# marinlauber/WaterLily

Hardware: AMD Instinct MI355X
Metric: MLUPS (cell-updates/s) per sim_step!, 3D sphere (higher is better)
Workload: dtype f32; 1 GPU; 3D sphere 512x512x512, Re=3700, f32, uniform inflow, remeasure=false (BASELINE configs[2]); layout=padded, transport=none, comm_ranks=1, scalar_allreduce=none

## Files before the change

### waterlily_amd/csrc/wl_api.hip

```cpp
#include <cstdarg>
#include <cstring>

#include <fcntl.h>
#include <sys/mman.h>
#include <sys/stat.h>
#include <unistd.h>

#include <rccl/rccl.h>

#include "wl_ops.h"
#include "wl_coarse.h"
#include "wl_measure.h"
#include "wl_mesh.h"
#include "wl_stats.h"
#include "wl_probe.h"
#include "wl_integrals.h"

namespace wl {

struct RcclComm : Comm {
    ncclComm_t nc = nullptr;
    ncclComm_t nch = nullptr;
    ~RcclComm() override {
        if (nch) ncclCommDestroy(nch);
// ... 177 lines not shown
};

Scratch &global_scratch(int *rc) {
    static Scratch s;
    static bool ok = false;
    *rc = 0;
    if (!ok) { *rc = s.init(); ok = (*rc == 0); }
    return s;
}

}

using namespace wl;

struct wl_mg {
    wl_dtype t;
    int D;
    int nlev;
    int permask;
    std::vector<wl_level_desc> lev;
    Scratch sc;
    std::vector<void *> rowc;
    unsigned char *dirty = nullptr;
    bool log_on = false;
    std::vector<double> log;
    int alloc_rowc() {
        const size_t es = t == WL_F32 ? 4 : 8;
        rowc.assign(nlev, nullptr);
        for (int l = 0; l < nlev; ++l) {
            const wl_grid &g = lev[l].g;
            if (g.D != 3) continue;
            WL_HIP(wl_dev_alloc(&rowc[l], (size_t)g.n[1] * (size_t)g.n[2] * RC_N * es));
        }
        return 0;
    }
    void free_scratch() {
        for (void *p : rowc) if (p) (void)hipFree(p);
        rowc.clear();
        if (dirty) (void)hipFree(dirty);
        dirty = nullptr;
    }
};
struct wl_flow {
    wl_dtype t;
    wl_flow_desc d;
    Scratch sc;
    unsigned char *rowfree = nullptr;
    unsigned char *rowbuf = nullptr;
    unsigned char *segbuf = nullptr;
    bool seg_valid = false;
    const unsigned char *segfree() const { return (seg_valid && opt(WL_OPT_BDIM_ROWFLAGS)) ? segbuf : nullptr; }
    int *busy = nullptr;
    int nbusy = 0;
    int nbusy_lo = 0, nbusy_hi = 0;
    size_t busy_cap = 0;
    int *rowcount = nullptr;
    long *rowoff = nullptr;
    unsigned char *touched = nullptr, *prev = nullptr;
    unsigned char *changed = nullptr;
    bool changed_valid = false;
    bool changed_pending = false;
    bool prev_valid = false;
    long nband = -1;
};

template <class T> static LevelT<T> lvl(const wl_mg *m, int l) {
    const wl_level_desc &d = m->lev[l];
    LevelT<T> o;
    o.g = mkG(&d.g);
    o.L = (T *)d.L; o.D = (T *)d.D; o.iD = (T *)d.iD; o.x = (T *)d.x; o.eps = (T *)d.eps; o.r = (T *)d.r; o.z = (T *)d.z;
    o.rowc = (opt(WL_OPT_ROW_CONST_L) && l < (int)m->rowc.size()) ? (const T *)m->rowc[l] : nullptr;
    return o;
}

template <class T, int D> static int mg_update(wl_mg *m, const unsigned char *dirty = nullptr) {
    {
        LevelT<T> p = lvl<T>(m, 0);
        WL_TRY((op_set_diag<T, D>(p.g, p.D, p.iD, p.L, dirty)));
        WL_TRY((halo_exchange<T>(p.g, p.iD, 1, 1)));
        if (D == 3 && m->rowc[0]) WL_TRY((op_lrow<T>(p.g, p.L, p.iD, (T *)m->rowc[0], dirty)));
    }
    for (int l = 1; l < m->nlev; ++l) {
        LevelT<T> a = lvl<T>(m, l), b = lvl<T>(m, l - 1);
        WL_TRY((op_restrictL<T, D>(a.g, a.L, b.g, b.L, m->permask)));
        WL_TRY((coarse_L_finish<T, D>(a.g, a.L, b.g, m->permask)));
        WL_TRY((op_set_diag<T, D>(a.g, a.D, a.iD, a.L)));
        WL_TRY((halo_exchange<T>(a.g, a.iD, 1, 1)));
        if (D == 3 && m->rowc[l]) WL_TRY((op_lrow<T>(a.g, a.L, a.iD, (T *)m->rowc[l])));
    }
    return 0;
}

template <class T, int D> static int mg_vcycle(wl_mg *m, int l, int *pcg_np = nullptr) {
    LevelT<T> fine = lvl<T>(m, l), coarse = lvl<T>(m, l + 1);
    const bool fused = (m->permask == 0) && opt(WL_OPT_SMOOTH_FUSED);
    if (fused) WL_TRY((op_smooth_fused<T, D>(fine, fine.eps)));
    else WL_TRY((op_jacobi<T, D>(fine, 1, m->permask)));
    const bool zero_in_restrict = (m->permask == 0) && !coarse.g.dist && !fine.g.dist;
    WL_TRY((op_restrict<T, D>(coarse.g, coarse.r, fine.g, fused ? fine.eps : fine.r, zero_in_restrict ? coarse.x : (T *)nullptr)));
    if (ctx().comm && ctx().comm->size > 1 && fine.g.dist && !coarse.g.dist) {
        const int nzl = (fine.g.nzg - 2) / ctx().comm->size / 2;
        WL_TRY(ctx().comm->allgather(coarse.r + coarse.g.s[2], (size_t)nzl * coarse.g.s[2] * sizeof(T)));
    }
    if (!zero_in_restrict) {
        Prof p(WL_K_MISC, coarse.g.cells());
        WL_HIP(hipMemsetAsync(coarse.x, 0, (size_t)span(coarse.g) * sizeof(T), ctx().stream));
    }
    const long tail_cells = coarse_tail_cells();
    bool tail = tail_cells && fused && !coarse.g.dist && coarse.g.interior_cells() <= tail_cells && (m->nlev - (l + 1)) <= CV_MAXLEV;
    if (tail) {
        CoarseArgs<T> ca;
        ca.nlev = m->nlev - (l + 1);
        for (int q = 0; q < ca.nlev; ++q) {
            ca.lev[q] = lvl<T>(m, l + 1 + q);
            if (ca.lev[q].g.dist) tail = false;
        }
        if (tail) {
            Prof p(WL_K_SMOOTH, coarse.g.cells());
            if (opt(WL_OPT_COARSE_PCG_RESIDENT)) hipLaunchKernelGGL((k_coarse_vcycle<T, D, true>), dim3(1), dim3(CV_THREADS), 0, ctx().stream, ca);
            else hipLaunchKernelGGL((k_coarse_vcycle<T, D, false>), dim3(1), dim3(CV_THREADS), 0, ctx().stream, ca);
            WL_HIP(hipGetLastError());
        }
    }
    if (!tail) {
        int pre = -1;
        if (l + 2 < m->nlev) WL_TRY((mg_vcycle<T, D>(m, l + 1, pcg_np ? &pre : nullptr)));
        WL_TRY((op_pcg<T, D>(coarse, 6, m->permask, m->sc.partials, m->sc.st, false, pre)));
    }
    if (pcg_np) *pcg_np = -1;
    if (fused) return op_prolong_increment_fused<T, D>(fine, fine.eps, coarse.g, coarse.x, m->sc.partials, pcg_np);
    WL_TRY((op_prolongate<T, D>(fine.g, fine.eps, coarse.g, coarse.x)));
    return op_increment<T, D>(fine, m->permask);
}

template <class T, int D> static int mg_Linf(wl_mg *m, int l) {
    LevelT<T> p = lvl<T>(m, l);
    const T *r = p.r;
    return op_reduce<T, D>(p.g, WL_K_DOT, RED_MAX, 0.0, [=] __device__(long I) { const double v = (double)r[I]; return v < 0 ? -v : v; },
                           m->sc.partials, m->sc.st, 1, true);
}
template <class T, int D> static int mg_log_row(wl_mg *m, int n, bool have_r2) {
    if (!have_r2) WL_TRY((op_L2<T, D>(lvl<T>(m, 0), m->sc.partials, m->sc.st, false)));
    WL_TRY((mg_Linf<T, D>(m, 0)));
    WL_TRY(m->sc.fetch());
    m->log.push_back((double)n); m->log.push_back(m->sc.hst->out[1]); m->log.push_back(m->sc.hst->r2);
    return 0;
}
template <class T, int D> static int mg_solve(wl_mg *m, double tol, int itmx, int *n_iter, const T *divu = nullptr, const G *gu = nullptr,
                                              bool halo_begun = false) {
    LevelT<T> p = lvl<T>(m, 0);
    WL_TRY((op_residual<T, D>(p, m->permask, m->sc.partials, m->sc.st, divu, gu, halo_begun)));
    int n = 0;
    if (m->log_on) WL_TRY((mg_log_row<T, D>(m, 0, false)));
    while (n < itmx) {
        int pre = -1;
        if (m->nlev > 1) WL_TRY((mg_vcycle<T, D>(m, 0, &pre)));
        WL_TRY((op_pcg<T, D>(p, 6, m->permask, m->sc.partials, m->sc.st, true, pre, true)));
        WL_TRY((op_L2<T, D>(p, m->sc.partials, m->sc.st, true)));
        WL_TRY(m->sc.fetch());
        ++n;
        const double r2 = m->sc.hst->r2;
        if (m->log_on) WL_TRY((mg_log_row<T, D>(m, n, true)));
        if (r2 < tol) break;
    }
    WL_TRY((op_bc_per<T, D>(p.g, p.x, m->permask)));
    if (n_iter) *n_iter = n;
    return 0;
}

template <class T> static ScaleOp project_scale(double dt_, double w) {
    const bool dbl = (w != 1.0);
    return ScaleOp{dbl ? w * (double)(T)dt_ : (double)(T)dt_, false, dbl};
}
template <class T, int D> static int flow_project(wl_flow *a, wl_mg *b, double dt_, double w, int *n_iter, bool exchange_u = false,
                                                  bool head_done = false, const ScaleOp *tail_then = nullptr, const XBc<T> *xbc = nullptr,
                                                  bool *xdone = nullptr, T *uvel = nullptr) {
    const G g = mkG(&a->d.g);
    T *const uv = uvel ? uvel : (T *)a->d.u;
    LevelT<T> p = lvl<T>(b, 0);
    const ScaleOp sc = project_scale<T>(dt_, w);
// ... 821 lines not shown
                       m->dirty, gm.n[1], gm.n[2], (int)yper, (int)zper);
    WL_HIP(hipGetLastError());
    const unsigned char *dirty = m->dirty;
    WL_MG_DISPATCH((mg_update<T, DD>(m, dirty)));
}
int wl_mg_mult(wl_mg *m, int level, void *x) {
    WL_LEVEL_OK();
    WL_MG_DISPATCH((op_mult<T, DD>(lvl<T>(m, level), (T *)x, m->permask)));
}
int wl_mg_residual(wl_mg *m, int level) {
    WL_LEVEL_OK();
    WL_MG_DISPATCH((op_residual<T, DD>(lvl<T>(m, level), m->permask, m->sc.partials, m->sc.st)));
}
int wl_mg_increment(wl_mg *m, int level) {
    WL_LEVEL_OK();
    WL_MG_DISPATCH((op_increment<T, DD>(lvl<T>(m, level), m->permask)));
}
int wl_mg_jacobi(wl_mg *m, int level, int it) {
    WL_LEVEL_OK();
    WL_MG_DISPATCH((op_jacobi<T, DD>(lvl<T>(m, level), it, m->permask)));
}
int wl_mg_pcg(wl_mg *m, int level, int it, int *n_updates) {
    WL_LEVEL_OK();
    int rc = [&]() -> int { WL_MG_DISPATCH((op_pcg<T, DD>(lvl<T>(m, level), it, m->permask, m->sc.partials, m->sc.st, false, -1, level == 0))); }();
    if (rc) return rc;
    if (n_updates) {
        WL_TRY(m->sc.fetch());
        *n_updates = m->sc.hst->nupd;
    }
    return 0;
}
int wl_mg_uniform_rows(wl_mg *m, int level, long long *n_uniform, long long *n_rows) {
    WL_LEVEL_OK();
    if (!n_uniform || !n_rows) return fail(WL_E_ARG, "wl_mg_uniform_rows: null output", __FILE__, __LINE__);
    const wl_grid &g = m->lev[level].g;
    *n_uniform = 0;
    *n_rows = (long long)(g.n[1] - 2) * (g.D == 3 ? (g.own_hi > 0 ? g.own_hi - g.own_lo + 1 : g.n[2] - 2) : 1);
    if (g.D != 3 || level >= (int)m->rowc.size() || !m->rowc[level]) return 0;
    const size_t es = m->t == WL_F32 ? 4 : 8, cnt = (size_t)g.n[1] * g.n[2] * RC_N;
    std::vector<char> h(cnt * es);
    WL_HIP(hipMemcpyAsync(h.data(), m->rowc[level], cnt * es, hipMemcpyDeviceToHost, ctx().stream));
    WL_HIP(hipStreamSynchronize(ctx().stream));
    for (size_t r = 0; r < cnt; r += RC_N) {
        const double c = m->t == WL_F32 ? (double)reinterpret_cast<const float *>(h.data())[r] : reinterpret_cast<const double *>(h.data())[r];
        if (c == c) ++*n_uniform;
    }
    return 0;
// ... 430 lines not shown
```

### waterlily_amd/csrc/wl_ops.h

```cpp
#pragma once
#include "wl_common.h"
#include "wl_convdiff.h"
#include "wl_stencil7.h"

namespace wl {

struct State {
    double rho, alpha, beta;
    double shift;
    double r2;
    double out[4];
    double red[4];
    int active;
    int do_shift;
    int nupd;
    int r2_valid;
    int xpend;
    PcgS slots[2];
};

template <class T> struct LevelT {
    G g;
    T *L, *D, *iD, *x, *eps, *r, *z;
    const T *rowc = nullptr;
};

inline long span(const G &g) { return g.D == 3 ? (long)g.n[2] * g.s[2] : (long)g.n[1] * g.s[1]; }

template <class T, int D> int op_bc_vec_fused(const G &g, T *a, const double *A, int saveexit, int permask, bool skip_x = false);
template <class T> struct XBc { int on, saveexit; T U0; };
template <class T> __device__ __forceinline__ void xbc_apply(const XBc<T> &b, T *u, long o, long sc, int i, int n0, VecA<T> (&uv)[3]) {
    constexpr int V = VecA<T>::V;
    if (!b.on) return;
    if (i == 1) { uv[0].v[0] = b.U0; u[o - 1] = b.U0; u[o - 1 + sc] = uv[1].v[0]; u[o - 1 + 2 * sc] = uv[2].v[0]; }
    if (i + V - 1 == n0 - 2) {
        if (!b.saveexit) u[o + V] = b.U0;
        u[o + V + sc] = uv[1].v[V - 1]; u[o + V + 2 * sc] = uv[2].v[V - 1];
    }
}
template <class T, int D>
int op_bc_vec(const G &g, T *a, const double *A, int saveexit, int permask, bool skip_x = false) {
    if (opt(WL_OPT_BC_FUSED)) return op_bc_vec_fused<T, D>(g, a, A, saveexit, permask, skip_x);
    if (skip_x) return fail(WL_E_STATE, "BC!: x planes folded into the producer need the one-launch form", __FILE__, __LINE__);
    for (int c = 0; c < D; ++c)
        for (int j = 0; j < D; ++j) {
            T *ac = a + (long)c * g.sc;
            const long sj = g.s[j];
            const int N = (j == 2) ? g.nzg : g.n[j];
// ... 1050 lines not shown
    }
    if (!exchanged) WL_TRY((halo_exchange<T>(p.g, p.r, 1, 1)));
    return launch_range(WL_K_SMOOTH, r_inside(p.g), [=] __device__(int i, int j, int k) {
        const long I = q.g.at(i, j, k);
        T lo[D], hi[D];
_Pragma("unroll")
        for (int d = 0; d < D; ++d) { lo[d] = q.L[I + (long)d * q.g.sc]; hi[d] = q.L[I + q.g.s[d] + (long)d * q.g.sc]; }
        T dg = 0;
_Pragma("unroll")
        for (int d = 0; d < D; ++d) dg -= (lo[d] + hi[d]);
        const T e0 = q.r[I] * q.iD[I];
        T s = e0 * dg;
_Pragma("unroll")
        for (int d = 0; d < D; ++d) {
            const long sd = q.g.s[d];
            s += (q.r[I - sd] * q.iD[I - sd]) * lo[d] + (q.r[I + sd] * q.iD[I + sd]) * hi[d];
        }
        rout[I] = q.r[I] - s;
        q.x[I] = q.x[I] + e0;
    });
}
template <class T, int D>
int op_prolong_increment_fused(const LevelT<T> &p, const T *rin, const G &gc, const T *cx, double *partials = nullptr,
                               int *pcg_np = nullptr) {
    WL_TRY((halo_exchange<T>(gc, const_cast<T *>(cx), 1, 1)));
    const LevelT<T> q = p;
    const G C = gc;
    if (pcg_np) *pcg_np = -1;
    if constexpr (D == 3) {
        if (stencil7_ok<T>(p.g)) {
            using VA = VecA<T>;
            const SrcProlong<T> src{cx, C, p.g.n[0], p.g.n[1], p.g.nzg, p.g.kz0};
            if (pcg_np && partials && opt(WL_OPT_PCG_START_FUSED) && opt(WL_OPT_PCG_RECOMPUTE_PRECOND) && opt(WL_OPT_PCG_VEC)) {
                T *e0 = p.eps;
                const int tpp = (((p.g.n[0] - 2 + 64 * VA::V - 1) / (64 * VA::V)) * ((p.g.n[1] - 2 + 3) / 4) + 7) / 8 * 8;
                Gate gcap;
                if (tpp <= WL_PCG_PARTIALS) gcap.zcap = WL_PCG_PARTIALS / tpp;
                int np = 0;
                const int rcv = launch_stencil7<T, 1>(WL_K_PROLONG, p.g, src, p.L, p.rowc, rin, p.x,
                    [=] __device__(long o, int i, int, int, const VA &ae, const VA &ec, const VA &r0, const VA &x0, const auto &rk, double *acc, const Pre &) {
                        VA rv = r0, xv = x0;
                        const VA id = row_iD<T>(rk, q.iD, o, i, q.g.n[0]);
_Pragma("unroll")
                        for (int v = 0; v < VA::V; ++v) { rv.v[v] = rv.v[v] - ae.v[v]; xv.v[v] = xv.v[v] + ec.v[v]; }
                        rv.store(q.r + o);
                        xv.store(q.x + o);
                        VA ev;
_Pragma("unroll")
                        for (int v = 0; v < VA::V; ++v) { ev.v[v] = rv.v[v] * id.v[v]; acc[0] += (double)rv.v[v] * (double)ev.v[v]; }
                        ev.store(e0 + o);
                    }, partials, &np, gcap);
                if (rcv > 0) return rcv;
                if (rcv == 0) { *pcg_np = np; return 0; }
            }
            const int rcv = launch_stencil7<T, 0>(WL_K_PROLONG, p.g, src, p.L, p.rowc, rin, p.x,
                [=] __device__(long o, int, int, int, const VA &ae, const VA &ec, const VA &r0, const VA &x0, const auto &, double *, const Pre &) {
                    VA rv = r0, xv = x0;
// ... 44 lines not shown
        : form(f), st(st_), partials(partials_), dist(dist_), xdef(xdef_), want_r2(want_r2_), eps10(eps10_), f32(sizeof(T) == 4), zcap(zcap_) {
        const bool own = f != PcgForm::FINALIZE;
        P0 = partials; PA = own ? partials + WL_MAXB : partials; PB = own ? partials + 2 * WL_MAXB : partials;
    }
    Gate base() const { Gate g; g.eps10 = (double)eps10; g.f32 = f32; g.zcap = zcap; return g; }
    int ready(const double *&part, int &n) const {
        if (form != PcgForm::SLAB) return 0;
        Prof pr(WL_K_SCALAR, 0);
        WL_TRY((reduce_allreduce<1>(part, n, (int)RED_SUM, 0.0, st->red)));
        part = st->red;
        n = 1;
        return 0;
    }
    int after_init(int np) const {
        if (form != PcgForm::FINALIZE) return 0;
        State *s = st;
        const T e10 = eps10;
        return launch_finalize<1>(dist, partials, np, RED_SUM, 0.0, st->red, [=] __device__(const double *v) {
            const T rho = (T)v[0];
            s->rho = (double)rho;
            s->nupd = 0;
            s->r2_valid = 0;
            s->xpend = 0;
            s->active = !((rho < 0 ? -rho : rho) < e10);
        });
    }
    int gate_mult(int n, int np0, Gate &g) {
        g = base();
        if (form == PcgForm::FINALIZE) { g.active = &st->active; return 0; }
        if (n == 1) {
            const double *gp = P0; int gn = np0;
            WL_TRY(ready(gp, gn));
            g.kind = 1; g.part = gp; g.np = gn; g.out = &st->slots[0]; cur = 0;
        } else { g.kind = 4; g.in = &st->slots[cur]; }
        return 0;
    }
    int after_mult(int np) const {
        if (form != PcgForm::FINALIZE) return 0;
        State *s = st;
        return launch_finalize<1>(dist, partials, np, RED_SUM, 0.0, st->red, [=] __device__(const double *v) {
            s->xpend = 0;
            if (!s->active) return;
            const T alpha = (T)s->rho / (T)v[0];
            const double aa = (double)(alpha < 0 ? -alpha : alpha);
            s->alpha = (double)alpha;
            if (aa < 1e-2 || aa > 1e2) s->active = 0;
        });
    }
    int gate_update(int npA, Gate &g) {
        g = base();
        if (form == PcgForm::FINALIZE) { g.active = &st->active; g.s0 = &st->alpha; return 0; }
        const double *gp = PA; int gn = npA;
        WL_TRY(ready(gp, gn));
        g.kind = 2; g.part = gp; g.np = gn; g.in = &st->slots[cur]; g.out = &st->slots[cur ^ 1];
        return 0;
    }
    void launched_update() { if (form != PcgForm::FINALIZE) cur ^= 1; }
    int after_update(int np, bool last, bool xnow) const {
        State *s = st;
        const bool wr2 = want_r2;
        if (form != PcgForm::FINALIZE) {
            if (!last) return 0;
            const int cs = cur;
            return launch_finalize<1>(dist, PB, np, RED_SUM, 0.0, st->red, [=] __device__(const double *v) {
                PcgS sl = s->slots[cs];
                if (sl.active) {
                    sl.nupd += 1;
                    if (wr2) { sl.r2 = (double)(T)v[0]; sl.r2_valid = 1; }
                    sl.active = 0;
                }
                s->rho = sl.rho; s->alpha = sl.alpha; s->beta = sl.beta;
                s->active = sl.active; s->xpend = sl.xpend; s->nupd = sl.nupd;
                s->r2_valid = sl.r2_valid;
                if (sl.r2_valid) s->r2 = sl.r2;
            });
        }
        const T e10 = eps10;
        return launch_finalize<1>(dist, partials, np, RED_SUM, 0.0, st->red, [=] __device__(const double *v) {
            if (!s->active) return;
            s->nupd += 1;
            if (last) {
                if (wr2) { s->r2 = (double)(T)v[0]; s->r2_valid = 1; }
                s->active = 0;
                return;
            }
            const T rho2 = (T)v[0];
            if ((rho2 < 0 ? -rho2 : rho2) < e10) { s->active = 0; s->xpend = !xnow; return; }
            s->beta = (double)(rho2 / (T)s->rho);
            s->rho = (double)rho2;
        });
    }
    int gate_direction(int npB, Gate &g) {
        g = base();
        if (form == PcgForm::FINALIZE) {
            g.active = &st->active; g.also = xdef ? &st->xpend : nullptr; g.s0 = &st->alpha; g.s1 = &st->beta;
            return 0;
        }
        const double *gp = PB; int gn = npB;
        WL_TRY(ready(gp, gn));
        g.kind = 3; g.part = gp; g.np = gn; g.in = &st->slots[cur]; g.out = &st->slots[cur ^ 1]; g.also_x = 1;
        return 0;
    }
    void launched_direction() { if (form != PcgForm::FINALIZE) cur ^= 1; }
};

inline bool pcg_recompute_aeps(long cells) {
    const int v = opt(WL_OPT_PCG_RECOMPUTE_AEPS);
    return v == 2 || (v == 3 && cells < (1L << 26)) || (v == 1 && cells < (1L << 26) && cells >= (1L << 22));
}
inline bool pcg_dots_in_kernel(long cells, bool distr) {
    const int v = opt(WL_OPT_PCG_DOTS_IN_KERNEL);
    return distr ? v != 0 : (v == 2 || (v == 1 && cells <= (1L << 25)));
}

template <class T, int D>
int op_pcg(const LevelT<T> &p, int it, int permask, double *partials, State *st, bool want_r2 = false,
           int pre_np = -1,
           bool ghost_z = false) {
    const LevelT<T> q = p;
    const Range R = r_inside(p.g);
    using VA = VecA<T>;
    const int n0 = p.g.n[0];
    bool vec = false;
    if constexpr (D == 3) vec = pcg_vec_ok<T>(p.g);
    const bool xdef = opt(WL_OPT_PCG_DEFER_X) != 0;
    const bool zrec = opt(WL_OPT_PCG_RECOMPUTE_PRECOND) != 0;
    bool zst = false;
    if constexpr (D == 3) zst = pcg_recompute_aeps(R.count()) && vec && zrec;
    const int tpp_v = D == 3 ? (((p.g.n[0] - 2 + 64 * VA::V - 1) / (64 * VA::V)) * ((p.g.n[1] - 2 + 3) / 4) + 7) / 8 * 8 : 0;
    const bool distr = p.g.dist && ctx().comm && ctx().comm->size > 1;
    const bool gates = vec && xdef && zrec && R.count() > 0 && tpp_v > 0 && pcg_dots_in_kernel(R.count(), distr) &&
                       (distr || tpp_v <= WL_PCG_PARTIALS);
    const PcgForm form = !gates ? PcgForm::FINALIZE : (distr ? PcgForm::SLAB : PcgForm::IN_KERNEL);
    const int zcap = form == PcgForm::IN_KERNEL ? std::max(WL_PCG_PARTIALS / std::max(tpp_v, 1), 1) : 0;
    PcgDots<T> dots(form, st, partials, p.g.dist, xdef, want_r2, (T)10 * Lim<T>::eps, zcap);
    const bool own = form != PcgForm::FINALIZE;
    int np = 0, np0 = 0, npA = 0;

    int rv0 = -1;
    if (pre_np >= 0) { rv0 = 0; np = np0 = pre_np; }
    else if (vec) {
        Gate gate_init = dots.base();
        rv0 = launch_rowvec<T, 1, true>(WL_K_PCG_INIT, p.g,
            [=] __device__(long o, int, int, const Pre &) { return VA::load(q.r + o); },
            [=] __device__(long o, int i, int, int, const VA &rr, const auto &rk, double *acc, const Pre &) {
                const VA id = row_iD<T>(rk, q.iD, o, i, n0);
                VA zv;
_Pragma("unroll")
                for (int v = 0; v < VA::V; ++v) { zv.v[v] = rr.v[v] * id.v[v]; acc[0] += (double)rr.v[v] * (double)zv.v[v]; }
                if (!zrec) zv.store(q.z + o);
                zv.store(q.eps + o);
            }, p.rowc, dots.P0, &np, gate_init);
        if (rv0 > 0) return rv0;
        np0 = np;
    }
    if (own && rv0 != 0) return fail(WL_E_STATE, "pcg: vector init kernel rejected", __FILE__, __LINE__);
    if (rv0 != 0)
    WL_TRY((launch_range_red<1>(WL_K_PCG_INIT, R, [=] __device__(int i, int j, int k, double(&acc)[1]) {
        const long I = q.g.at(i, j, k);
        const T v = q.r[I] * q.iD[I];
        if (!zrec) q.z[I] = v;
        q.eps[I] = v;
        acc[0] += (double)q.r[I] * (double)v;
    }, partials, RED_SUM, 0.0, &np)));
    WL_TRY(dots.after_init(np));

    for (int n = 1; n <= it; ++n) {
        const bool last = (n == it);
        const bool xnow = last || !xdef;
        WL_TRY((op_bc_per<T, D>(p.g, p.eps, permask, false)));
        bool exchanged = false;
        int rcv = -1;
        if constexpr (D == 3) {
            if (stencil7_ok<T>(p.g)) {
                exchanged = true;
                Gate gate_mult;
                WL_TRY(dots.gate_mult(n, np0, gate_mult));
                rcv = launch_stencil7_halo<T, 1>(WL_K_PCG_MULT, p.g, p.eps, SrcArray<T>{p.eps}, p.L, p.rowc, (const T *)nullptr, (const T *)nullptr,
                    [=] __device__(long o, int, int, int, const VA &ae, const VA &ec, const VA &, const VA &, const auto &, double *acc, const Pre &) {
                    if (!zst) ae.store(q.z + o);
_Pragma("unroll")
                    for (int v = 0; v < VA::V; ++v) acc[0] += (double)ae.v[v] * (double)ec.v[v];
                }, dots.PA, &np, gate_mult);
                if (rcv > 0) return rcv;
                if (own && rcv != 0) return fail(WL_E_STATE, "pcg: vector mult kernel rejected", __FILE__, __LINE__);
            }
        }
        if (!exchanged) WL_TRY((halo_exchange<T>(p.g, p.eps, 1, 1)));
        if (rcv != 0)
        WL_TRY((launch_range_red<1>(WL_K_PCG_MULT, R, [=] __device__(int i, int j, int k, double(&acc)[1]) {
            if (!st->active) return;
            const long I = q.g.at(i, j, k);
            const T v = mult1r<T, D>(q.g, q.L, q.eps, I);
            q.z[I] = v;
            acc[0] += (double)v * (double)q.eps[I];
        }, partials, RED_SUM, 0.0, &np)));
        if (ghost_z && permask != 0) {
            int planes = 0, nps = 0;
            for (int j = 0; j < D; ++j) if ((permask >> j) & 1) planes |= 3 << (2 * j);
            const G gg = p.g;
            WL_TRY((launch_shell_red(WL_K_PCG_MULT, p.g, planes, [=] __device__(int i, int j, int k, double(&acc)[1]) {
                const long I = gg.at(i, j, k);
                acc[0] += (double)q.z[I] * (double)q.eps[I];
            }, (rcv == 0 ? dots.PA : partials) + np, RED_SUM, 0.0, &nps, own ? 32 : 256)));
            np += nps;
        }
        npA = np;
        WL_TRY(dots.after_mult(np));

        int rvu = -1;
        Gate gate_upd;
        WL_TRY(dots.gate_update(npA, gate_upd));
        if constexpr (D == 3) {
            if (zst) {
                auto upd_epi = [=] __device__(long o, int i, int, int, const VA &ae, const VA &ec, const VA &r0, const VA &x0, const auto &rk, double *acc, const Pre &pre) {
                    const T alpha = (T)pre.s0;
                    VA rr = r0;
                    if (xnow) {
                        VA xv = x0;
_Pragma("unroll")
                        for (int v = 0; v < VA::V; ++v) xv.v[v] += alpha * ec.v[v];
                        xv.store(q.x + o);
                    }
_Pragma("unroll")
                    for (int v = 0; v < VA::V; ++v) rr.v[v] = rr.v[v] - alpha * ae.v[v];
                    rr.store(q.r + o);
                    if (!last) {
                        const VA id = row_iD<T>(rk, q.iD, o, i, n0);
_Pragma("unroll")
                        for (int v = 0; v < VA::V; ++v) { const T zn = rr.v[v] * id.v[v]; acc[0] += (double)rr.v[v] * (double)zn; }
                    } else if (want_r2) {
_Pragma("unroll")
                        for (int v = 0; v < VA::V; ++v) acc[0] += (double)rr.v[v] * (double)rr.v[v];
                    }
                };
                const T *xin = xnow ? (const T *)q.x : (const T *)nullptr;
                rvu = launch_stencil7<T, 1>(WL_K_PCG_UPDATE, p.g, SrcArray<T>{p.eps}, p.L, p.rowc, (const T *)q.r, xin, upd_epi, dots.PB, &np, gate_upd);
                if (rvu != 0) return rvu > 0 ? rvu : fail(WL_E_STATE, "pcg: 7-point update kernel rejected", __FILE__, __LINE__);
                dots.launched_update();
            }
        }
        if (vec && rvu != 0) {
            struct UD { VA r, z, x, e; };
            rvu = launch_rowvec<T, 1, true>(WL_K_PCG_UPDATE, p.g,
                [=] __device__(long o, int, int, const Pre &) {
                    UD d;
                    d.r = VA::load(q.r + o);
                    d.z = VA::load(q.z + o);
                    if (xnow) { d.x = VA::load(q.x + o); d.e = VA::load(q.eps + o); }
                    return d;
                },
                [=] __device__(long o, int i, int, int, const UD &d, const auto &rk, double *acc, const Pre &pre) {
                    const T alpha = (T)pre.s0;
                    VA rr = d.r;
                    if (xnow) {
                        VA xv = d.x;
_Pragma("unroll")
                        for (int v = 0; v < VA::V; ++v) xv.v[v] += alpha * d.e.v[v];
                        xv.store(q.x + o);
                    }
_Pragma("unroll")
                    for (int v = 0; v < VA::V; ++v) rr.v[v] = rr.v[v] - alpha * d.z.v[v];
                    rr.store(q.r + o);
                    if (!last) {
                        const VA id = row_iD<T>(rk, q.iD, o, i, n0);
                        VA zn;
_Pragma("unroll")
                        for (int v = 0; v < VA::V; ++v) { zn.v[v] = rr.v[v] * id.v[v]; acc[0] += (double)rr.v[v] * (double)zn.v[v]; }
                        if (!zrec) zn.store(q.z + o);
                    } else if (want_r2) {
_Pragma("unroll")
                        for (int v = 0; v < VA::V; ++v) acc[0] += (double)rr.v[v] * (double)rr.v[v];
                    }
                }, p.rowc, dots.PB, &np, gate_upd);
            if (rvu > 0) return rvu;
            if (own && rvu != 0) return fail(WL_E_STATE, "pcg: vector update kernel rejected", __FILE__, __LINE__);
            if (rvu == 0) dots.launched_update();
        }
        if (rvu != 0)
        WL_TRY((launch_range_red<1>(WL_K_PCG_UPDATE, R, [=] __device__(int i, int j, int k, double(&acc)[1]) {
            if (!st->active) return;
            const long I = q.g.at(i, j, k);
            const T alpha = (T)st->alpha;
            if (xnow) q.x[I] += alpha * q.eps[I];
            const T rn = q.r[I] - alpha * q.z[I];
            q.r[I] = rn;
            if (!last) {
                const T zn = rn * q.iD[I];
                if (!zrec) q.z[I] = zn;
                acc[0] += (double)rn * (double)zn;
            } else if (want_r2) {
                acc[0] += (double)rn * (double)rn;
            }
        }, partials, RED_SUM, 0.0, &np)));
        WL_TRY(dots.after_update(np, last, xnow));
        if (last) break;

        int rvd = -1;
        Gate gate_dir;
        WL_TRY(dots.gate_direction(np, gate_dir));
        if (vec) {
            struct DD { VA e, x, z; };
            rvd = launch_rowvec<T, 0, true>(WL_K_PCG_DIR, p.g,
                [=] __device__(long o, int, int, const Pre &pre) {
                    DD d;
                    d.e = VA::load(q.eps + o);
                    if (xdef) d.x = VA::load(q.x + o);
                    if (pre.act) d.z = VA::load((zrec ? q.r : q.z) + o);
                    return d;
                },
                [=] __device__(long o, int i, int, int, const DD &d, const auto &rk, double *, const Pre &pre) {
                    VA ev = d.e, zv = VA::splat((T)0);
                    if (pre.act) {
                        zv = d.z;
                        if (zrec) {
                            const VA id = row_iD<T>(rk, q.iD, o, i, n0);
_Pragma("unroll")
                            for (int v = 0; v < VA::V; ++v) zv.v[v] = d.z.v[v] * id.v[v];
                        }
                    }
                    if (xdef) {
                        const T alpha = (T)pre.s0;
                        VA xv = d.x;
_Pragma("unroll")
                        for (int v = 0; v < VA::V; ++v) xv.v[v] += alpha * ev.v[v];
                        xv.store(q.x + o);
                    }
                    if (!pre.act) return;
                    const T beta = (T)pre.s1;
_Pragma("unroll")
                    for (int v = 0; v < VA::V; ++v) ev.v[v] = beta * ev.v[v] + zv.v[v];
                    ev.store(q.eps + o);
                }, p.rowc, nullptr, nullptr, gate_dir);
            if (rvd > 0) return rvd;
            if (own && rvd != 0) return fail(WL_E_STATE, "pcg: vector direction kernel rejected", __FILE__, __LINE__);
            if (rvd == 0) dots.launched_direction();
        }
        if (rvd != 0)
        WL_TRY(launch_range(WL_K_PCG_DIR, R, [=] __device__(int i, int j, int k) {
            const int act = st->active;
            if (!act && !(xdef && st->xpend)) return;
            const long I = q.g.at(i, j, k);
            if (xdef) {
                q.x[I] += (T)st->alpha * q.eps[I];
                if (!act) return;
            }
            q.eps[I] = (T)st->beta * q.eps[I] + (zrec ? q.r[I] * q.iD[I] : q.z[I]);
        }));
    }
    return 0;
}

template <class T, int D>
int op_L2(const LevelT<T> &p, double *partials, State *st, bool after_pcg = false) {
    const LevelT<T> q = p;
    int np = 0;
    int rcv = -1;
    if constexpr (D == 3) {
        if (pcg_vec_ok<T>(p.g)) {
            using VA = VecA<T>;
            Gate gate;
            if (after_pcg) { gate.active = &st->r2_valid; gate.inv = 1; }
            rcv = launch_rowvec<T, 1, false>(WL_K_DOT, p.g,
                [=] __device__(long o, int, int, const Pre &) { return VA::load(q.r + o); },
                [=] __device__(long, int, int, int, const VA &rr, const auto &, double *acc, const Pre &) {
_Pragma("unroll")
                    for (int v = 0; v < VA::V; ++v) acc[0] += (double)rr.v[v] * (double)rr.v[v];
// ... 92 lines not shown
```

### waterlily_amd/csrc/wl_stencil7.h

```cpp
#pragma once
#include <type_traits>

#include "wl_common.h"

namespace wl {

typedef float wl_f4u __attribute__((ext_vector_type(4), aligned(4)));
typedef double wl_d2u __attribute__((ext_vector_type(2), aligned(8)));
template <class T> struct Vec16;
template <> struct Vec16<float> { static constexpr int V = 4; using type = wl_f4u; };
template <> struct Vec16<double> { static constexpr int V = 2; using type = wl_d2u; };

template <class T> struct VecA {
    static constexpr int V = Vec16<T>::V;
    T v[V];
    __device__ __forceinline__ static VecA load(const T *p) {
        VecA r;
        const typename Vec16<T>::type q = *reinterpret_cast<const typename Vec16<T>::type *>(p);
        __builtin_memcpy(r.v, &q, 16);
        return r;
    }
    __device__ __forceinline__ void store(T *p) const {
        typename Vec16<T>::type q;
        __builtin_memcpy(&q, v, 16);
        *reinterpret_cast<typename Vec16<T>::type *>(p) = q;
    }
    __device__ __forceinline__ static VecA splat(T x) {
        VecA r;
#pragma unroll
        for (int q = 0; q < V; ++q) r.v[q] = x;
        return r;
    }
};

constexpr int S7_BY = 4;

struct PcgS { double rho, alpha, beta, r2; int active, xpend, nupd, r2_valid; };
struct Gate {
    const int *active = nullptr, *also = nullptr;
    const double *s0 = nullptr, *s1 = nullptr;
    int kind = 0;
    const double *part = nullptr;
    int np = 0;
    const PcgS *in = nullptr;
    PcgS *out = nullptr;
    double eps10 = 0.0;
    int f32 = 1;
    int also_x = 0;
    int inv = 0;
    int rev = 0;
    int zcap = 0;
};
constexpr int WL_PCG_PARTIALS = 1024;
struct Pre { int act; double s0, s1; };
__device__ __forceinline__ double pcg_rnd(double x, int f32) { return f32 ? (double)(float)x : x; }
__device__ __forceinline__ double pcg_div(double a, double b, int f32) { return f32 ? (double)((float)a / (float)b) : a / b; }
__device__ __forceinline__ void pcg_after_init(PcgS &s, double v, double eps10, int f32) {
    const double rho = pcg_rnd(v, f32);
    s.rho = rho; s.alpha = 0.0; s.beta = 0.0; s.r2 = 0.0;
    s.nupd = 0; s.r2_valid = 0; s.xpend = 0;
    s.active = !((rho < 0 ? -rho : rho) < eps10);
}
__device__ __forceinline__ void pcg_after_mult(PcgS &s, double v, int f32) {
    s.xpend = 0;
    if (!s.active) return;
    const double alpha = pcg_div(s.rho, pcg_rnd(v, f32), f32);
    const double aa = alpha < 0 ? -alpha : alpha;
    s.alpha = alpha;
    if (aa < 1e-2 || aa > 1e2) s.active = 0;
}
__device__ __forceinline__ void pcg_after_update(PcgS &s, double v, double eps10, int f32, bool xnow) {
    if (!s.active) return;
    s.nupd += 1;
    const double rho2 = pcg_rnd(v, f32);
    if ((rho2 < 0 ? -rho2 : rho2) < eps10) { s.active = 0; s.xpend = !xnow; return; }
    s.beta = pcg_div(rho2, s.rho, f32);
    s.rho = rho2;
}
__device__ __forceinline__ double block_sum_partials(const double *part, int np) {
    __shared__ double bc;
    double acc[1] = {0.0};
    for (int i = threadIdx.x; i < np; i += 256) acc[0] = acc[0] + part[i];
    block_red<1>(acc, RED_SUM);
    if (threadIdx.x == 0) bc = acc[0];
    __syncthreads();
    return bc;
}
__device__ __forceinline__ bool gate_open(const Gate &gt, Pre &pre) {
    pre.act = 1; pre.s0 = 0.0; pre.s1 = 0.0;
    bool run = true;
    if (gt.kind == 0) {
        if (gt.active) { pre.act = gt.inv ? !*gt.active : *gt.active; run = pre.act || (gt.also && *gt.also); }
        if (gt.s0) pre.s0 = *gt.s0;
        if (gt.s1) pre.s1 = *gt.s1;
        return run;
    }
    PcgS s;
    if (gt.kind == 1) {
        pcg_after_init(s, block_sum_partials(gt.part, gt.np), gt.eps10, gt.f32);
    } else {
        s = *gt.in;
        if (gt.kind == 2) pcg_after_mult(s, block_sum_partials(gt.part, gt.np), gt.f32);
        else if (gt.kind == 3) pcg_after_update(s, block_sum_partials(gt.part, gt.np), gt.eps10, gt.f32, false);
    }
    if (gt.out && blockIdx.x == 0 && threadIdx.x == 0) *gt.out = s;
    pre.act = s.active; pre.s0 = s.alpha; pre.s1 = s.beta;
    return s.active || (gt.also_x && s.xpend);
}

constexpr int RC_N = 8;
template <class T> struct RowK {
    T c, idc, idf, idl, lxf, lxl;
    __device__ __forceinline__ bool uni() const { return c == c; }
};
template <class T> struct RowKU : RowK<T> {
    __device__ __forceinline__ RowKU(const RowK<T> &r) : RowK<T>(r) {}
    __device__ __forceinline__ constexpr bool uni() const { return true; }
};
template <class T> __device__ __forceinline__ RowK<T> rowk_none() {
    RowK<T> r;
    r.c = __builtin_nanf("");
    r.idc = r.idf = r.idl = r.lxf = r.lxl = (T)0;
    return r;
}
template <class T> __device__ __forceinline__ RowK<T> rowk_load(const T *rowc, long row) {
    if (!rowc) return rowk_none<T>();
    typedef T wl_rc8 __attribute__((ext_vector_type(8)));
    typedef const __attribute__((address_space(4))) wl_rc8 *cptr;
    const wl_rc8 a = *(cptr)(rowc + RC_N * row);
    RowK<T> r;
// ... 452 lines not shown
```

Before: 5657 MLUPS.

## Defer PCG solution updates via a ring of stored search directions

Adds an optional PCG mode that writes each iteration's search direction into its own ring buffer and records the alphas in device-side state. The solution x is then updated once, in the final update kernel, with all accumulated alpha·e terms, instead of reading and writing x in every iteration. This is meant to cut per-iteration memory traffic on x. The cost is extra device memory per multigrid level, larger gate and Pre structs, and FMA contraction turned off in the x axpy paths to keep rounding consistent between modes. Under the usual default option value the ring mode appears to stay off.

Result: slower. 5584 MLUPS (-1.3%).

```diff
diff --git a/waterlily_amd/csrc/wl_api.hip b/waterlily_amd/csrc/wl_api.hip
--- a/waterlily_amd/csrc/wl_api.hip
+++ b/waterlily_amd/csrc/wl_api.hip
@@ -223,6 +223,8 @@
     Scratch sc;
     std::vector<void *> rowc;
     unsigned char *dirty = nullptr;
+    std::vector<void *> ring;
+    std::vector<int> ring_state;
     bool log_on = false;
     std::vector<double> log;
     int alloc_rowc() {
@@ -238,6 +240,9 @@
     void free_scratch() {
         for (void *p : rowc) if (p) (void)hipFree(p);
         rowc.clear();
+        for (void *p : ring) if (p) (void)hipFree(p);
+        ring.clear();
+        ring_state.clear();
         if (dirty) (void)hipFree(dirty);
         dirty = nullptr;
     }
@@ -274,6 +279,25 @@
     return o;
 }
 
+template <class T, int D> static int mg_ring(wl_mg *m, int l, int it, PcgRing<T> *out) {
+    *out = PcgRing<T>();
+    const G g = mkG(&m->lev[l].g);
+    if (!opt(WL_OPT_PCG_DEFER_X) || !pcg_ring_ok<T, D>(g, it, m->permask)) return 0;
+    if ((int)m->ring.size() != m->nlev) { m->ring.assign(m->nlev, nullptr); m->ring_state.assign(m->nlev, 0); }
+    const size_t n = (size_t)span(g);
+    if (m->ring_state[l] == 0) {
+        void *blk = nullptr;
+        const size_t bytes = n * sizeof(T) * (WL_PCG_RING - 1);
+        if (wl_dev_alloc(&blk, bytes) != hipSuccess || !blk) { (void)hipGetLastError(); m->ring_state[l] = -1; return 0; }
+        m->ring[l] = blk;
+        m->ring_state[l] = 1;
+        WL_HIP(hipMemsetAsync(blk, 0, bytes, ctx().stream));
+    }
+    if (m->ring_state[l] != 1) return 0;
+    for (int k = 0; k < WL_PCG_RING - 1; ++k) out->s[k] = (T *)m->ring[l] + n * k;
+    return 0;
+}
+
 template <class T, int D> static int mg_update(wl_mg *m, const unsigned char *dirty = nullptr) {
     {
         LevelT<T> p = lvl<T>(m, 0);
@@ -290,6 +314,12 @@
         if (D == 3 && m->rowc[l]) WL_TRY((op_lrow<T>(a.g, a.L, a.iD, (T *)m->rowc[l])));
     }
     return 0;
+}
+
+template <class T, int D> static int mg_pcg(wl_mg *m, int l, int it) {
+    PcgRing<T> rg;
+    WL_TRY((mg_ring<T, D>(m, l, it, &rg)));
+    return op_pcg<T, D>(lvl<T>(m, l), it, m->permask, m->sc.partials, m->sc.st, false, -1, l == 0, &rg);
 }
 
 template <class T, int D> static int mg_vcycle(wl_mg *m, int l, int *pcg_np = nullptr) {
@@ -326,10 +356,16 @@
     if (!tail) {
         int pre = -1;
         if (l + 2 < m->nlev) WL_TRY((mg_vcycle<T, D>(m, l + 1, pcg_np ? &pre : nullptr)));
-        WL_TRY((op_pcg<T, D>(coarse, 6, m->permask, m->sc.partials, m->sc.st, false, pre)));
+        PcgRing<T> rg;
+        WL_TRY((mg_ring<T, D>(m, l + 1, 6, &rg)));
+        WL_TRY((op_pcg<T, D>(coarse, 6, m->permask, m->sc.partials, m->sc.st, false, pre, false, &rg)));
     }
     if (pcg_np) *pcg_np = -1;
-    if (fused) return op_prolong_increment_fused<T, D>(fine, fine.eps, coarse.g, coarse.x, m->sc.partials, pcg_np);
+    if (fused) {
+        PcgRing<T> rg;
+        if (pcg_np) WL_TRY((mg_ring<T, D>(m, l, 6, &rg)));
+        return op_prolong_increment_fused<T, D>(fine, fine.eps, coarse.g, coarse.x, m->sc.partials, pcg_np, rg.s[0]);
+    }
     WL_TRY((op_prolongate<T, D>(fine.g, fine.eps, coarse.g, coarse.x)));
     return op_increment<T, D>(fine, m->permask);
 }
@@ -356,7 +392,9 @@
     while (n < itmx) {
         int pre = -1;
         if (m->nlev > 1) WL_TRY((mg_vcycle<T, D>(m, 0, &pre)));
-        WL_TRY((op_pcg<T, D>(p, 6, m->permask, m->sc.partials, m->sc.st, true, pre, true)));
+        PcgRing<T> rg;
+        WL_TRY((mg_ring<T, D>(m, 0, 6, &rg)));
+        WL_TRY((op_pcg<T, D>(p, 6, m->permask, m->sc.partials, m->sc.st, true, pre, true, &rg)));
         WL_TRY((op_L2<T, D>(p, m->sc.partials, m->sc.st, true)));
         WL_TRY(m->sc.fetch());
         ++n;
@@ -1224,7 +1262,7 @@
 }
 int wl_mg_pcg(wl_mg *m, int level, int it, int *n_updates) {
     WL_LEVEL_OK();
-    int rc = [&]() -> int { WL_MG_DISPATCH((op_pcg<T, DD>(lvl<T>(m, level), it, m->permask, m->sc.partials, m->sc.st, false, -1, level == 0))); }();
+    int rc = [&]() -> int { WL_MG_DISPATCH((mg_pcg<T, DD>(m, level, it))); }();
     if (rc) return rc;
     if (n_updates) {
         WL_TRY(m->sc.fetch());
diff --git a/waterlily_amd/csrc/wl_ops.h b/waterlily_amd/csrc/wl_ops.h
--- a/waterlily_amd/csrc/wl_ops.h
+++ b/waterlily_amd/csrc/wl_ops.h
@@ -16,6 +16,7 @@
     int nupd;
     int r2_valid;
     int xpend;
+    PcgRingS rs;
     PcgS slots[2];
 };
 
@@ -24,6 +25,16 @@
     T *L, *D, *iD, *x, *eps, *r, *z;
     const T *rowc = nullptr;
 };
+
+template <class T> struct PcgRing {
+    T *s[WL_PCG_RING - 1] = {nullptr, nullptr, nullptr, nullptr, nullptr};
+    bool on() const { return s[0] != nullptr; }
+};
+template <class T> __host__ __device__ __forceinline__ T pcg_axpy(T alpha, T e, T x) {
+#pragma clang fp contract(off)
+    const T ae = alpha * e;
+    return x + ae;
+}
 
 inline long span(const G &g) { return g.D == 3 ? (long)g.n[2] * g.s[2] : (long)g.n[1] * g.s[1]; }
 
@@ -1120,7 +1131,7 @@
 }
 template <class T, int D>
 int op_prolong_increment_fused(const LevelT<T> &p, const T *rin, const G &gc, const T *cx, double *partials = nullptr,
-                               int *pcg_np = nullptr) {
+                               int *pcg_np = nullptr, T *pcg_e1 = nullptr) {
     WL_TRY((halo_exchange<T>(gc, const_cast<T *>(cx), 1, 1)));
     const LevelT<T> q = p;
     const G C = gc;
@@ -1130,7 +1141,7 @@
             using VA = VecA<T>;
             const SrcProlong<T> src{cx, C, p.g.n[0], p.g.n[1], p.g.nzg, p.g.kz0};
             if (pcg_np && partials && opt(WL_OPT_PCG_START_FUSED) && opt(WL_OPT_PCG_RECOMPUTE_PRECOND) && opt(WL_OPT_PCG_VEC)) {
-                T *e0 = p.eps;
+                T *e0 = pcg_e1 ? pcg_e1 : p.eps;
                 const int tpp = (((p.g.n[0] - 2 + 64 * VA::V - 1) / (64 * VA::V)) * ((p.g.n[1] - 2 + 3) / 4) + 7) / 8 * 8;
                 Gate gcap;
                 if (tpp <= WL_PCG_PARTIALS) gcap.zcap = WL_PCG_PARTIALS / tpp;
@@ -1221,6 +1232,7 @@
             s->nupd = 0;
             s->r2_valid = 0;
             s->xpend = 0;
+            pcg_ring_reset(s->rs);
             s->active = !((rho < 0 ? -rho : rho) < e10);
         });
     }
@@ -1244,11 +1256,13 @@
             const double aa = (double)(alpha < 0 ? -alpha : alpha);
             s->alpha = (double)alpha;
             if (aa < 1e-2 || aa > 1e2) s->active = 0;
+            else pcg_ring_owe(s->rs, (double)alpha);
         });
     }
-    int gate_update(int npA, Gate &g) {
+    int gate_update(int npA, Gate &g, bool ring_last = false) {
         g = base();
-        if (form == PcgForm::FINALIZE) { g.active = &st->active; g.s0 = &st->alpha; return 0; }
+        g.always = ring_last;
+        if (form == PcgForm::FINALIZE) { g.active = &st->active; g.s0 = &st->alpha; if (ring_last) g.rs = &st->rs; return 0; }
         const double *gp = PA; int gn = npA;
         WL_TRY(ready(gp, gn));
         g.kind = 2; g.part = gp; g.np = gn; g.in = &st->slots[cur]; g.out = &st->slots[cur ^ 1];
@@ -1270,7 +1284,7 @@
                 }
                 s->rho = sl.rho; s->alpha = sl.alpha; s->beta = sl.beta;
                 s->active = sl.active; s->xpend = sl.xpend; s->nupd = sl.nupd;
-                s->r2_valid = sl.r2_valid;
+                s->r2_valid = sl.r2_valid; s->rs = sl.rs;
                 if (sl.r2_valid) s->r2 = sl.r2;
             });
         }
@@ -1287,17 +1301,18 @@
             if ((rho2 < 0 ? -rho2 : rho2) < e10) { s->active = 0; s->xpend = !xnow; return; }
             s->beta = (double)(rho2 / (T)s->rho);
             s->rho = (double)rho2;
+            s->rs.ndir += 1;
         });
     }
-    int gate_direction(int npB, Gate &g) {
+    int gate_direction(int npB, Gate &g, bool ring = false) {
         g = base();
         if (form == PcgForm::FINALIZE) {
-            g.active = &st->active; g.also = xdef ? &st->xpend : nullptr; g.s0 = &st->alpha; g.s1 = &st->beta;
+            g.active = &st->active; g.also = (xdef && !ring) ? &st->xpend : nullptr; g.s0 = &st->alpha; g.s1 = &st->beta;
             return 0;
         }
         const double *gp = PB; int gn = npB;
         WL_TRY(ready(gp, gn));
-        g.kind = 3; g.part = gp; g.np = gn; g.in = &st->slots[cur]; g.out = &st->slots[cur ^ 1]; g.also_x = 1;
+        g.kind = 3; g.part = gp; g.np = gn; g.in = &st->slots[cur]; g.out = &st->slots[cur ^ 1]; g.also_x = !ring;
         return 0;
     }
     void launched_direction() { if (form != PcgForm::FINALIZE) cur ^= 1; }
@@ -1312,10 +1327,26 @@
     return distr ? v != 0 : (v == 2 || (v == 1 && cells <= (1L << 25)));
 }
 
+constexpr int WL_PCG_RING_DEFAULT = 2;
+inline bool pcg_ring_range(long cells) {
+    int v = opt(WL_OPT_PCG_DEFER_X);
+    if (v == 1) v = WL_PCG_RING_DEFAULT;
+    return v == 3 || (v == 4 && cells > (1L << 25));
+}
+template <class T, int D> inline bool pcg_ring_ok(const G &g, int it, int permask) {
+    if constexpr (D != 3) return false;
+    else {
+        const long cells = r_inside(g).count();
+        return it >= 2 && it <= WL_PCG_RING && permask == 0 && !g.dist && cells > 0 && pcg_vec_ok<T>(g) && rowvec_fits<T>(g) &&
+               opt(WL_OPT_PCG_RECOMPUTE_PRECOND) != 0 && !pcg_recompute_aeps(cells) && pcg_ring_range(cells);
+    }
+}
+
 template <class T, int D>
 int op_pcg(const LevelT<T> &p, int it, int permask, double *partials, State *st, bool want_r2 = false,
            int pre_np = -1,
-           bool ghost_z = false) {
+           bool ghost_z = false,
+           const PcgRing<T> *ringp = nullptr) {
     const LevelT<T> q = p;
     const Range R = r_inside(p.g);
     using VA = VecA<T>;
@@ -1326,6 +1357,10 @@
     const bool zrec = opt(WL_OPT_PCG_RECOMPUTE_PRECOND) != 0;
     bool zst = false;
     if constexpr (D == 3) zst = pcg_recompute_aeps(R.count()) && vec && zrec;
+    const bool ring = ringp && ringp->on() && xdef && pcg_ring_ok<T, D>(p.g, it, permask);
+    if (ringp && ringp->on() && !ring) return fail(WL_E_STATE, "pcg: ring arrays given to a call that cannot use them", __FILE__, __LINE__);
+    T *em[WL_PCG_RING + 1];
+    for (int n = 1; n <= WL_PCG_RING; ++n) em[n] = (ring && n < it) ? ringp->s[n - 1] : p.eps;
     const int tpp_v = D == 3 ? (((p.g.n[0] - 2 + 64 * VA::V - 1) / (64 * VA::V)) * ((p.g.n[1] - 2 + 3) / 4) + 7) / 8 * 8 : 0;
     const bool distr = p.g.dist && ctx().comm && ctx().comm->size > 1;
     const bool gates = vec && xdef && zrec && R.count() > 0 && tpp_v > 0 && pcg_dots_in_kernel(R.count(), distr) &&
@@ -1339,6 +1374,7 @@
     int rv0 = -1;
     if (pre_np >= 0) { rv0 = 0; np = np0 = pre_np; }
     else if (vec) {
+        T *const e1 = em[1];
         Gate gate_init = dots.base();
         rv0 = launch_rowvec<T, 1, true>(WL_K_PCG_INIT, p.g,
             [=] __device__(long o, int, int, const Pre &) { return VA::load(q.r + o); },
@@ -1348,12 +1384,12 @@
 _Pragma("unroll")
                 for (int v = 0; v < VA::V; ++v) { zv.v[v] = rr.v[v] * id.v[v]; acc[0] += (double)rr.v[v] * (double)zv.v[v]; }
                 if (!zrec) zv.store(q.z + o);
-                zv.store(q.eps + o);
+                zv.store(e1 + o);
             }, p.rowc, dots.P0, &np, gate_init);
         if (rv0 > 0) return rv0;
         np0 = np;
     }
-    if (own && rv0 != 0) return fail(WL_E_STATE, "pcg: vector init kernel rejected", __FILE__, __LINE__);
+    if ((own || ring) && rv0 != 0) return fail(WL_E_STATE, "pcg: vector init kernel rejected", __FILE__, __LINE__);
     if (rv0 != 0)
     WL_TRY((launch_range_red<1>(WL_K_PCG_INIT, R, [=] __device__(int i, int j, int k, double(&acc)[1]) {
         const long I = q.g.at(i, j, k);
@@ -1367,7 +1403,8 @@
     for (int n = 1; n <= it; ++n) {
         const bool last = (n == it);
         const bool xnow = last || !xdef;
-        WL_TRY((op_bc_per<T, D>(p.g, p.eps, permask, false)));
+        T *const en = em[n];
+        WL_TRY((op_bc_per<T, D>(p.g, en, permask, false)));
         bool exchanged = false;
         int rcv = -1;
         if constexpr (D == 3) {
@@ -1375,14 +1412,14 @@
                 exchanged = true;
                 Gate gate_mult;
                 WL_TRY(dots.gate_mult(n, np0, gate_mult));
-                rcv = launch_stencil7_halo<T, 1>(WL_K_PCG_MULT, p.g, p.eps, SrcArray<T>{p.eps}, p.L, p.rowc, (const T *)nullptr, (const T *)nullptr,
+                rcv = launch_stencil7_halo<T, 1>(WL_K_PCG_MULT, p.g, en, SrcArray<T>{en}, p.L, p.rowc, (const T *)nullptr, (const T *)nullptr,
                     [=] __device__(long o, int, int, int, const VA &ae, const VA &ec, const VA &, const VA &, const auto &, double *acc, const Pre &) {
                     if (!zst) ae.store(q.z + o);
 _Pragma("unroll")
                     for (int v = 0; v < VA::V; ++v) acc[0] += (double)ae.v[v] * (double)ec.v[v];
                 }, dots.PA, &np, gate_mult);
                 if (rcv > 0) return rcv;
-                if (own && rcv != 0) return fail(WL_E_STATE, "pcg: vector mult kernel rejected", __FILE__, __LINE__);
+                if ((own || ring) && rcv != 0) return fail(WL_E_STATE, "pcg: vector mult kernel rejected", __FILE__, __LINE__);
             }
         }
         if (!exchanged) WL_TRY((halo_exchange<T>(p.g, p.eps, 1, 1)));
@@ -1409,7 +1446,54 @@
 
         int rvu = -1;
         Gate gate_upd;
-        WL_TRY(dots.gate_update(npA, gate_upd));
+        WL_TRY(dots.gate_update(npA, gate_upd, ring && last));
+        if (ring && last) {
+            struct UR { VA r, z, x, e[WL_PCG_RING]; };
+            struct EP { const T *e[WL_PCG_RING]; } ep;
+            for (int k = 0; k < WL_PCG_RING; ++k) ep.e[k] = em[k + 1];
+            rvu = launch_rowvec<T, 1, false>(WL_K_PCG_UPDATE, p.g,
+                [=] __device__(long o, int, int, const Pre &) {
+                    UR d;
+                    d.r = VA::load(q.r + o);
+                    d.z = VA::load(q.z + o);
+                    d.x = VA::load(q.x + o);
+_Pragma("unroll")
+                    for (int k = 0; k < WL_PCG_RING; ++k) d.e[k] = VA::load(ep.e[k] + o);
+                    return d;
+                },
+                [=] __device__(long o, int, int, int, const UR &d, const auto &, double *acc, const Pre &pre) {
+                    const int nx = pre.rs.nx;
+                    VA xv = d.x;
+_Pragma("unroll")
+                    for (int k = 0; k < WL_PCG_RING; ++k) {
+                        const T ak = (T)pre.rs.al[k];
+_Pragma("unroll")
+                        for (int v = 0; v < VA::V; ++v) { const T xn = pcg_axpy(ak, d.e[k].v[v], xv.v[v]); xv.v[v] = k < nx ? xn : xv.v[v]; }
+                    }
+                    if (nx > 0) xv.store(q.x + o);
+                    if (!pre.act) {
+                        const int nd = pre.rs.ndir;
+                        if (nd < it) {
+                            VA ev = d.e[0];
+_Pragma("unroll")
+                            for (int k = 1; k < WL_PCG_RING; ++k) if (k == nd - 1) ev = d.e[k];
+                            ev.store(q.eps + o);
+                        }
+                        return;
+                    }
+                    const T alpha = (T)pre.s0;
+                    VA rr = d.r;
+_Pragma("unroll")
+                    for (int v = 0; v < VA::V; ++v) rr.v[v] = rr.v[v] - alpha * d.z.v[v];
+                    rr.store(q.r + o);
+                    if (want_r2) {
+_Pragma("unroll")
+                        for (int v = 0; v < VA::V; ++v) acc[0] += (double)rr.v[v] * (double)rr.v[v];
+                    }
+                }, p.rowc, dots.PB, &np, gate_upd);
+            if (rvu != 0) return rvu > 0 ? rvu : fail(WL_E_STATE, "pcg: ring update kernel rejected", __FILE__, __LINE__);
+            dots.launched_update();
+        }
         if constexpr (D == 3) {
             if (zst) {
                 auto upd_epi = [=] __device__(long o, int i, int, int, const VA &ae, const VA &ec, const VA &r0, const VA &x0, const auto &rk, double *acc, const Pre &pre) {
@@ -1418,7 +1502,7 @@
                     if (xnow) {
                         VA xv = x0;
 _Pragma("unroll")
-                        for (int v = 0; v < VA::V; ++v) xv.v[v] += alpha * ec.v[v];
+                        for (int v = 0; v < VA::V; ++v) xv.v[v] = pcg_axpy(alpha, ec.v[v], xv.v[v]);
                         xv.store(q.x + o);
                     }
 _Pragma("unroll")
@@ -1441,21 +1525,22 @@
         }
         if (vec && rvu != 0) {
             struct UD { VA r, z, x, e; };
+            const bool xk = xnow && !ring;
             rvu = launch_rowvec<T, 1, true>(WL_K_PCG_UPDATE, p.g,
                 [=] __device__(long o, int, int, const Pre &) {
                     UD d;
                     d.r = VA::load(q.r + o);
                     d.z = VA::load(q.z + o);
-                    if (xnow) { d.x = VA::load(q.x + o); d.e = VA::load(q.eps + o); }
+                    if (xk) { d.x = VA::load(q.x + o); d.e = VA::load(q.eps + o); }
                     return d;
                 },
                 [=] __device__(long o, int i, int, int, const UD &d, const auto &rk, double *acc, const Pre &pre) {
                     const T alpha = (T)pre.s0;
                     VA rr = d.r;
-                    if (xnow) {
+                    if (xk) {
                         VA xv = d.x;
 _Pragma("unroll")
-                        for (int v = 0; v < VA::V; ++v) xv.v[v] += alpha * d.e.v[v];
+                        for (int v = 0; v < VA::V; ++v) xv.v[v] = pcg_axpy(alpha, d.e.v[v], xv.v[v]);
                         xv.store(q.x + o);
                     }
 _Pragma("unroll")
@@ -1473,7 +1558,7 @@
                     }
                 }, p.rowc, dots.PB, &np, gate_upd);
             if (rvu > 0) return rvu;
-            if (own && rvu != 0) return fail(WL_E_STATE, "pcg: vector update kernel rejected", __FILE__, __LINE__);
+            if ((own || ring) && rvu != 0) return fail(WL_E_STATE, "pcg: vector update kernel rejected", __FILE__, __LINE__);
             if (rvu == 0) dots.launched_update();
         }
         if (rvu != 0)
@@ -1481,7 +1566,7 @@
             if (!st->active) return;
             const long I = q.g.at(i, j, k);
             const T alpha = (T)st->alpha;
-            if (xnow) q.x[I] += alpha * q.eps[I];
+            if (xnow) q.x[I] = pcg_axpy(alpha, q.eps[I], q.x[I]);
             const T rn = q.r[I] - alpha * q.z[I];
             q.r[I] = rn;
             if (!last) {
@@ -1497,8 +1582,30 @@
 
         int rvd = -1;
         Gate gate_dir;
-        WL_TRY(dots.gate_direction(np, gate_dir));
-        if (vec) {
+        WL_TRY(dots.gate_direction(np, gate_dir, ring));
+        if (ring) {
+            struct DR { VA e, r; };
+            const T *ein = en;
+            T *const eout = em[n + 1];
+            rvd = launch_rowvec<T, 0, true>(WL_K_PCG_DIR, p.g,
+                [=] __device__(long o, int, int, const Pre &) {
+                    DR d;
+                    d.e = VA::load(ein + o);
+                    d.r = VA::load(q.r + o);
+                    return d;
+                },
+                [=] __device__(long o, int i, int, int, const DR &d, const auto &rk, double *, const Pre &pre) {
+                    const VA id = row_iD<T>(rk, q.iD, o, i, n0);
+                    const T beta = (T)pre.s1;
+                    VA ev;
+_Pragma("unroll")
+                    for (int v = 0; v < VA::V; ++v) { const T zv = d.r.v[v] * id.v[v]; ev.v[v] = beta * d.e.v[v] + zv; }
+                    ev.store(eout + o);
+                }, p.rowc, nullptr, nullptr, gate_dir);
+            if (rvd != 0) return rvd > 0 ? rvd : fail(WL_E_STATE, "pcg: ring direction kernel rejected", __FILE__, __LINE__);
+            dots.launched_direction();
+        }
+        if (vec && rvd != 0) {
             struct DD { VA e, x, z; };
             rvd = launch_rowvec<T, 0, true>(WL_K_PCG_DIR, p.g,
                 [=] __device__(long o, int, int, const Pre &pre) {
@@ -1522,7 +1629,7 @@
                         const T alpha = (T)pre.s0;
                         VA xv = d.x;
 _Pragma("unroll")
-                        for (int v = 0; v < VA::V; ++v) xv.v[v] += alpha * ev.v[v];
+                        for (int v = 0; v < VA::V; ++v) xv.v[v] = pcg_axpy(alpha, ev.v[v], xv.v[v]);
                         xv.store(q.x + o);
                     }
                     if (!pre.act) return;
@@ -1541,7 +1648,7 @@
             if (!act && !(xdef && st->xpend)) return;
             const long I = q.g.at(i, j, k);
             if (xdef) {
-                q.x[I] += (T)st->alpha * q.eps[I];
+                q.x[I] = pcg_axpy((T)st->alpha, q.eps[I], q.x[I]);
                 if (!act) return;
             }
             q.eps[I] = (T)st->beta * q.eps[I] + (zrec ? q.r[I] * q.iD[I] : q.z[I]);
diff --git a/waterlily_amd/csrc/wl_stencil7.h b/waterlily_amd/csrc/wl_stencil7.h
--- a/waterlily_amd/csrc/wl_stencil7.h
+++ b/waterlily_amd/csrc/wl_stencil7.h
@@ -35,7 +35,9 @@
 
 constexpr int S7_BY = 4;
 
-struct PcgS { double rho, alpha, beta, r2; int active, xpend, nupd, r2_valid; };
+constexpr int WL_PCG_RING = 6;
+struct PcgRingS { double al[WL_PCG_RING]; int nx, ndir; };
+struct PcgS { double rho, alpha, beta, r2; int active, xpend, nupd, r2_valid; PcgRingS rs; };
 struct Gate {
     const int *active = nullptr, *also = nullptr;
     const double *s0 = nullptr, *s1 = nullptr;
@@ -47,18 +49,31 @@
     double eps10 = 0.0;
     int f32 = 1;
     int also_x = 0;
+    const PcgRingS *rs = nullptr;
+    int always = 0;
     int inv = 0;
     int rev = 0;
     int zcap = 0;
 };
 constexpr int WL_PCG_PARTIALS = 1024;
-struct Pre { int act; double s0, s1; };
+struct Pre { int act; double s0, s1; PcgRingS rs; };
 __device__ __forceinline__ double pcg_rnd(double x, int f32) { return f32 ? (double)(float)x : x; }
 __device__ __forceinline__ double pcg_div(double a, double b, int f32) { return f32 ? (double)((float)a / (float)b) : a / b; }
+__device__ __forceinline__ void pcg_ring_reset(PcgRingS &rs) {
+#pragma unroll
+    for (int k = 0; k < WL_PCG_RING; ++k) rs.al[k] = 0.0;
+    rs.nx = 0; rs.ndir = 1;
+}
+__device__ __forceinline__ void pcg_ring_owe(PcgRingS &rs, double alpha) {
+#pragma unroll
+    for (int k = 0; k < WL_PCG_RING; ++k) if (k == rs.nx) rs.al[k] = alpha;
+    if (rs.nx < WL_PCG_RING) rs.nx += 1;
+}
 __device__ __forceinline__ void pcg_after_init(PcgS &s, double v, double eps10, int f32) {
     const double rho = pcg_rnd(v, f32);
     s.rho = rho; s.alpha = 0.0; s.beta = 0.0; s.r2 = 0.0;
     s.nupd = 0; s.r2_valid = 0; s.xpend = 0;
+    pcg_ring_reset(s.rs);
     s.active = !((rho < 0 ? -rho : rho) < eps10);
 }
 __device__ __forceinline__ void pcg_after_mult(PcgS &s, double v, int f32) {
@@ -68,6 +83,7 @@
     const double aa = alpha < 0 ? -alpha : alpha;
     s.alpha = alpha;
     if (aa < 1e-2 || aa > 1e2) s.active = 0;
+    else pcg_ring_owe(s.rs, alpha);
 }
 __device__ __forceinline__ void pcg_after_update(PcgS &s, double v, double eps10, int f32, bool xnow) {
     if (!s.active) return;
@@ -76,6 +92,7 @@
     if ((rho2 < 0 ? -rho2 : rho2) < eps10) { s.active = 0; s.xpend = !xnow; return; }
     s.beta = pcg_div(rho2, s.rho, f32);
     s.rho = rho2;
+    s.rs.ndir += 1;
 }
 __device__ __forceinline__ double block_sum_partials(const double *part, int np) {
     __shared__ double bc;
@@ -88,11 +105,13 @@
 }
 __device__ __forceinline__ bool gate_open(const Gate &gt, Pre &pre) {
     pre.act = 1; pre.s0 = 0.0; pre.s1 = 0.0;
+    pre.rs.nx = 0; pre.rs.ndir = 0;
     bool run = true;
     if (gt.kind == 0) {
-        if (gt.active) { pre.act = gt.inv ? !*gt.active : *gt.active; run = pre.act || (gt.also && *gt.also); }
+        if (gt.active) { pre.act = gt.inv ? !*gt.active : *gt.active; run = pre.act || (gt.also && *gt.also) || gt.always; }
         if (gt.s0) pre.s0 = *gt.s0;
         if (gt.s1) pre.s1 = *gt.s1;
+        if (gt.rs) pre.rs = *gt.rs;
         return run;
     }
     PcgS s;
@@ -104,8 +123,8 @@
         else if (gt.kind == 3) pcg_after_update(s, block_sum_partials(gt.part, gt.np), gt.eps10, gt.f32, false);
     }
     if (gt.out && blockIdx.x == 0 && threadIdx.x == 0) *gt.out = s;
-    pre.act = s.active; pre.s0 = s.alpha; pre.s1 = s.beta;
-    return s.active || (gt.also_x && s.xpend);
+    pre.act = s.active; pre.s0 = s.alpha; pre.s1 = s.beta; pre.rs = s.rs;
+    return s.active || (gt.also_x && s.xpend) || gt.always;
 }
 
 constexpr int RC_N = 8;
```
